# ethanshenley/Neural-Collaborative-Filtering-Demo

Measured on AMD Instinct MI355X. Metric: train samples/sec + infer pairs/sec, 1M×100K d=64 AdvancedNCF @1/2/4/8 GPU, higher is better.
Workload: dtype fp32; 1 GPU; C2 train step: 1M users x 100K items, D=64, H=4, MLP [256,128,64], T=32, dropout 0.2, Adam lr 1e-3 wd 1e-5 (dense-exact); global_batch=20480, groups_per_gpu=4096, samples_per_group=5, launch=host launches, parallelism=single-gpu

## Files before the change

neural-collaborative-filtering-demo_amd/csrc/dedup.hip:

```cpp
#include "segments.h"

using namespace ncf_seg;

namespace {

constexpr uint32_t ST_AGG = 1u << 30, ST_INCL = 2u << 30, ST_MASK = (1u << 30) - 1;
constexpr int kDirectTiles = 64;

__device__ __forceinline__ uint32_t ld_status(const uint32_t* p) {
  return __hip_atomic_load(p, __ATOMIC_RELAXED, __HIP_MEMORY_SCOPE_AGENT);
}
__device__ __forceinline__ void st_status(uint32_t* p, uint32_t v) {
  __hip_atomic_store(p, v, __ATOMIC_RELAXED, __HIP_MEMORY_SCOPE_AGENT);
}
__device__ __forceinline__ uint64_t ld_status64(const uint64_t* p) {
  return __hip_atomic_load(p, __ATOMIC_RELAXED, __HIP_MEMORY_SCOPE_AGENT);
}
__device__ __forceinline__ void st_status64(uint64_t* p, uint64_t v) {
  __hip_atomic_store(p, v, __ATOMIC_RELAXED, __HIP_MEMORY_SCOPE_AGENT);
}

__device__ __forceinline__ uint32_t clamp_key(int64_t id, int64_t rows) {
  return (id < 0 || id >= rows) ? 0u : (uint32_t)id;
}

__global__ __launch_bounds__(256) void k_keys_hist(
    const int64_t* __restrict__ ids0, int64_t rows0, const int64_t* __restrict__ ids1,
    int64_t rows1, int64_t n0, int64_t n1, int bits, int passes, uint32_t* __restrict__ k0,
    uint32_t* __restrict__ v0, uint32_t* __restrict__ k1, uint32_t* __restrict__ v1,
    uint32_t* __restrict__ ghist, uint32_t* __restrict__ num_unique, uint32_t* __restrict__ start0,
    uint32_t* __restrict__ start1, uint32_t* __restrict__ pstart0, uint32_t* __restrict__ pstart1,
    uint32_t* __restrict__ fpiece0, uint32_t* __restrict__ fpiece1) {
  __shared__ uint32_t h[MAXP][MAXR];
  const int kind = blockIdx.y;
  const int64_t n = kind ? n1 : n0;
  const int64_t rows = kind ? rows1 : rows0;
  const int64_t* ids = kind ? ids1 : ids0;
  uint32_t* k = kind ? k1 : k0;
  uint32_t* v = kind ? v1 : v0;
  const int R = 1 << bits;
  if (n == 0) {
    if (blockIdx.x == 0 && threadIdx.x == 0) {
      if (num_unique) num_unique[kind] = 0;
      (kind ? start1 : start0)[0] = 0;
      (kind ? pstart1 : pstart0)[0] = 0;
      (kind ? fpiece1 : fpiece0)[0] = 0;
    }
    return;
  }
  if ((int64_t)blockIdx.x * TILE >= n) return;
  for (int i = threadIdx.x; i < passes * MAXR; i += 256) (&h[0][0])[i] = 0;
  __syncthreads();
#pragma unroll
  for (int r = 0; r < 4; ++r) {
    const int64_t i = (int64_t)blockIdx.x * TILE + r * 256 + threadIdx.x;
    if (i < n) {
      const uint32_t key = clamp_key(ids[i], rows);
      k[i] = key;
      v[i] = (uint32_t)i;
      for (int p = 0; p < passes; ++p) atomicAdd(&h[p][(key >> (p * bits)) & (R - 1)], 1u);
    }
  }
  __syncthreads();
  for (int p = 0; p < passes; ++p)
    for (int d = threadIdx.x; d < R; d += 256)
      if (h[p][d]) atomicAdd(&ghist[((int64_t)p * 2 + kind) * MAXR + d], h[p][d]);
}

__global__ __launch_bounds__(256) void k_onesweep(
    const uint32_t* __restrict__ kin0, const uint32_t* __restrict__ vin0,
    const uint32_t* __restrict__ kin1, const uint32_t* __restrict__ vin1, int64_t n0, int64_t n1,
    int shift, int bits, const uint32_t* __restrict__ ghist, uint32_t* __restrict__ status,
    int nbmax, uint32_t* __restrict__ tickets, uint32_t* __restrict__ kout0,
    uint32_t* __restrict__ vout0, uint32_t* __restrict__ kout1, uint32_t* __restrict__ vout1) {
  __shared__ uint32_t wcnt[4][MAXR];
  __shared__ uint32_t tcnt[MAXR];
  __shared__ uint32_t base[MAXR];
  __shared__ uint32_t csum[256];
  __shared__ uint32_t s_tile;
  const int kind = blockIdx.y;
  const int64_t n = kind ? n1 : n0;
  if (n == 0) return;
  const int nb = (int)((n + TILE - 1) / TILE);
  const int R = 1 << bits;
  const int tid = threadIdx.x, lane = tid & 63, w = tid >> 6;
  if (tid == 0) s_tile = atomicAdd(&tickets[kind], 1u);
  for (int i = tid; i < 4 * R; i += 256) wcnt[i / R][i % R] = 0;
  __syncthreads();
  const int tile = (int)s_tile;
  if (tile >= nb) return;
  const uint32_t* kin = kind ? kin1 : kin0;
  const uint32_t* vin = kind ? vin1 : vin0;
  uint32_t* kout = kind ? kout1 : kout0;
  uint32_t* vout = kind ? vout1 : vout0;
  uint32_t* st = status + ((int64_t)kind * nbmax) * R;

  const int64_t kb = (int64_t)tile * TILE + w * 256;
  uint32_t key[4], val[4], dig[4], loc[4];
  bool ok[4];
  const uint64_t lt = (lane == 0) ? 0ull : ((~0ull) >> (64 - lane));
#pragma unroll
  for (int it = 0; it < 4; ++it) {
    const int64_t i = kb + it * 64 + lane;
    ok[it] = i < n;
    key[it] = ok[it] ? kin[i] : 0u;
    val[it] = ok[it] ? vin[i] : 0u;
    dig[it] = (key[it] >> shift) & (uint32_t)(R - 1);
    uint64_t peers = __ballot(ok[it]);
    for (int b = 0; b < bits; ++b) {
      const uint64_t bb = __ballot((dig[it] >> b) & 1u);
      peers &= ((dig[it] >> b) & 1u) ? bb : ~bb;
    }
    const uint32_t before = (uint32_t)__popcll(peers & lt);
    uint32_t c = 0;
    if (ok[it]) c = wcnt[w][dig[it]];
    __builtin_amdgcn_wave_barrier();
    loc[it] = c + before;
    if (ok[it] && before == 0) wcnt[w][dig[it]] = c + (uint32_t)__popcll(peers);
    __builtin_amdgcn_wave_barrier();
  }
  __syncthreads();
  for (int d = tid; d < R; d += 256) {
    uint32_t run = 0;
#pragma unroll
    for (int ww = 0; ww < 4; ++ww) {
      const uint32_t c = wcnt[ww][d];
      wcnt[ww][d] = run;
      run += c;
    }
    tcnt[d] = run;
    st_status(&st[(int64_t)tile * R + d], (tile == 0 ? ST_INCL : ST_AGG) | run);
  }
  const uint32_t* gh = ghist + (int64_t)kind * MAXR;
  const int per = (R + 255) / 256;
  uint32_t mine = 0;
  for (int j = 0; j < per; ++j) {
    const int d = tid * per + j;
    if (d < R) mine += gh[d];
  }
  csum[tid] = mine;
  __syncthreads();
  for (int off = 1; off < 256; off <<= 1) {
    const uint32_t x = tid >= off ? csum[tid - off] : 0u;
    __syncthreads();
    csum[tid] += x;
    __syncthreads();
  }
  {
    uint32_t run = csum[tid] - mine;
    for (int j = 0; j < per; ++j) {
      const int d = tid * per + j;
      if (d < R) {
        base[d] = run;
        run += gh[d];
      }
    }
  }
  __syncthreads();
  if (nb <= kDirectTiles) {
    const uint64_t* st64 = reinterpret_cast<const uint64_t*>(st);
    for (int d0 = 2 * tid; d0 < R; d0 += 512) {
      uint32_t e0 = 0, e1 = 0;
      for (int tb = 0; tb < tile; tb += 8) {
        uint64_t v[8];
#pragma unroll
        for (int j = 0; j < 8; ++j)
          v[j] = tb + j < tile ? ld_status64(&st64[((int64_t)(tb + j) * R + d0) / 2])
                               : ((uint64_t)ST_AGG << 32 | ST_AGG);
#pragma unroll
        for (int j = 0; j < 8; ++j) {
          while (((uint32_t)v[j] & ~ST_MASK) == 0 || ((uint32_t)(v[j] >> 32) & ~ST_MASK) == 0) {
            __builtin_amdgcn_s_sleep(1);
            v[j] = ld_status64(&st64[((int64_t)(tb + j) * R + d0) / 2]);
          }
          e0 += (uint32_t)v[j] & ST_MASK;
          e1 += (uint32_t)(v[j] >> 32) & ST_MASK;
        }
      }
      base[d0] += e0;
      base[d0 + 1] += e1;
    }
  } else {
    for (int d = tid; d < R; d += 256) {
      uint32_t excl = 0;
      if (tile > 0) {
        int t = tile - 1;
        while (true) {
          const uint32_t s = ld_status(&st[(int64_t)t * R + d]);
          if ((s & ~ST_MASK) == 0) {
            __builtin_amdgcn_s_sleep(1);
            continue;
          }
          excl += s & ST_MASK;
          if (s & ST_INCL) break;
          --t;
        }
        st_status(&st[(int64_t)tile * R + d], ST_INCL | (excl + tcnt[d]));
      }
      base[d] += excl;
    }
  }
  __syncthreads();
#pragma unroll
  for (int it = 0; it < 4; ++it) {
    if (!ok[it]) continue;
    const uint32_t pos = base[dig[it]] + wcnt[w][dig[it]] + loc[it];
    kout[pos] = key[it];
    vout[pos] = val[it];
  }
}

__global__ __launch_bounds__(256) void k_segments(
    const uint32_t* __restrict__ sk0, const uint32_t* __restrict__ sk1, int64_t n0, int64_t n1,
    int nbmax, uint64_t* __restrict__ sstatus, uint32_t* __restrict__ tickets,
    uint32_t* __restrict__ segoff, uint32_t* __restrict__ start0, uint32_t* __restrict__ start1,
    uint32_t* __restrict__ pstart0, uint32_t* __restrict__ pstart1, uint32_t* __restrict__ pseg0,
    uint32_t* __restrict__ pseg1, uint32_t* __restrict__ fpiece0, uint32_t* __restrict__ fpiece1,
    int64_t* __restrict__ uniq0, int64_t* __restrict__ uniq1, int32_t* __restrict__ slot0,
    int32_t* __restrict__ slot1, uint32_t* __restrict__ totals, uint32_t* __restrict__ num_unique) {
  constexpr uint64_t F_AGG = 1ull << 62, F_INCL = 2ull << 62, M31 = (1ull << 31) - 1;
  __shared__ uint32_t ws_s[16], ws_p[16];
  __shared__ uint32_t s_tile, s_es, s_ep;
  const int kind = blockIdx.y;
  const int64_t n = kind ? n1 : n0;
  if (n == 0) return;
  const int nb = (int)((n + TILE - 1) / TILE);
  const int tid = threadIdx.x, lane = tid & 63, w = tid >> 6;
  if (tid == 0) s_tile = atomicAdd(&tickets[kind], 1u);
  __syncthreads();
  const int tile = (int)s_tile;
  if (tile >= nb) return;
  const uint32_t* sk = kind ? sk1 : sk0;
  uint64_t* st = sstatus + (int64_t)kind * nbmax;
  const uint64_t le = (lane == 63) ? ~0ull : ((1ull << (lane + 1)) - 1);
  bool sh[4], ph[4];
  uint32_t sr[4], pr[4], key[4];
#pragma unroll
  for (int r = 0; r < 4; ++r) {
    const int64_t i = (int64_t)tile * TILE + r * 256 + tid;
    key[r] = i < n ? sk[i] : 0u;
    sh[r] = i < n && (i == 0 || key[r] != sk[i - 1]);
    ph[r] = i < n && (sh[r] || (i % PIECE) == 0);
    const uint64_t ms = __ballot(sh[r]), mp = __ballot(ph[r]);
    sr[r] = (uint32_t)__popcll(ms & le);
    pr[r] = (uint32_t)__popcll(mp & le);
    if (lane == 0) {
      ws_s[r * 4 + w] = (uint32_t)__popcll(ms);
      ws_p[r * 4 + w] = (uint32_t)__popcll(mp);
    }
  }
  __syncthreads();
  if (w == 0) {
    uint64_t S = 0, Pc = 0;
    for (int q = 0; q < 16; ++q) { S += ws_s[q]; Pc += ws_p[q]; }
    uint64_t es = 0, ep = 0;
    if (nb <= kDirectTiles) {
      if (lane == 0) st_status64(&st[tile], F_AGG | (S << 31) | Pc);
      uint64_t v = 0;
      if (lane < tile) {
        do {
          v = ld_status64(&st[lane]);
          if ((v >> 62) == 0) __builtin_amdgcn_s_sleep(1);
        } while ((v >> 62) == 0);
      }
      uint32_t a = (uint32_t)((v >> 31) & M31), b = (uint32_t)(v & M31);
#pragma unroll
      for (int o = 32; o > 0; o >>= 1) {
        a += __shfl_xor(a, o, 64);
        b += __shfl_xor(b, o, 64);
      }
      es = a;
      ep = b;
    } else if (lane == 0) {
      if (tile == 0) {
        st_status64(&st[0], F_INCL | (S << 31) | Pc);
      } else {
        st_status64(&st[tile], F_AGG | (S << 31) | Pc);
        int t = tile - 1;
        while (true) {
          const uint64_t s = ld_status64(&st[t]);
          if ((s >> 62) == 0) {
            __builtin_amdgcn_s_sleep(1);
            continue;
          }
          es += (s >> 31) & M31;
          ep += s & M31;
          if (s & F_INCL) break;
          --t;
        }
// ... 155 lines not shown
}

static int64_t g_small_max = kSmallMax;

__global__ __launch_bounds__(256) void k_seg_inverse(const uint32_t* __restrict__ sk0,
                                                     const uint32_t* __restrict__ sk1,
                                                     const uint32_t* __restrict__ sv0,
                                                     const uint32_t* __restrict__ sv1, int64_t n0,
                                                     int64_t n1, int nb,
                                                     const uint32_t* __restrict__ off,
                                                     int64_t* __restrict__ inv0,
                                                     int64_t* __restrict__ inv1) {
  __shared__ uint32_t wsum[16];
  const int kind = blockIdx.y;
  const int64_t n = kind ? n1 : n0;
  const uint32_t* sk = kind ? sk1 : sk0;
  const uint32_t* sv = kind ? sv1 : sv0;
  int64_t* inv = kind ? inv1 : inv0;
  const int lane = threadIdx.x & 63, w = threadIdx.x >> 6;
  bool head[4];
  uint32_t rank[4];
  const uint64_t le = (lane == 63) ? ~0ull : ((1ull << (lane + 1)) - 1);
  for (int r = 0; r < 4; ++r) {
    const int64_t i = (int64_t)blockIdx.x * TILE + r * 256 + threadIdx.x;
    head[r] = i < n && (i == 0 || sk[i] != sk[i - 1]);
    const uint64_t m = __ballot(head[r]);
    rank[r] = (uint32_t)__popcll(m & le);
    if (lane == 0) wsum[r * 4 + w] = (uint32_t)__popcll(m);
  }
  __syncthreads();
  const uint32_t base = off[(int64_t)kind * nb + blockIdx.x];
  for (int r = 0; r < 4; ++r) {
    const int64_t i = (int64_t)blockIdx.x * TILE + r * 256 + threadIdx.x;
    if (i >= n) continue;
    uint32_t pre = 0;
    for (int q = 0; q < r * 4 + w; ++q) pre += wsum[q];
    inv[sv[i]] = (int64_t)(base + pre + rank[r]) - 1;
  }
}

}

extern "C" int ncf_dedup_ids2(const int64_t* ids0, int64_t n0, int64_t rows0, const int64_t* ids1,
                              int64_t n1, int64_t rows1, int64_t dim, int64_t* uniq0,
                              int64_t* uniq1, int32_t* slot0, int32_t* slot1,
                              uint32_t* num_unique, void* workspace, int64_t workspace_bytes,
                              void* stream) {
  const int64_t n = n0 > n1 ? n0 : n1;
  NCF_CHECK_ARG(n0 >= 0 && n1 >= 0 && n < (1ll << 30), "ncf_dedup_ids: bad n");
  NCF_CHECK_ARG(rows0 >= 1 && rows1 >= 1 && rows0 <= (1ll << 32) && rows1 <= (1ll << 32),
                "ncf_dedup_ids: rows must be in [1, 2^32]");
  if (workspace_bytes < ws_bytes(n, dim)) {
    ncf_set_error("ncf_dedup_ids: workspace %lld < %lld bytes", (long long)workspace_bytes,
                  (long long)ws_bytes(n, dim));
    return NCF_ERR_WORKSPACE;
  }
  hipStream_t st = (hipStream_t)stream;
  WS w = carve(workspace, n, dim);
  const int passes = sort_passes(rows0, rows1), bits = digit_bits(rows0, rows1);
  if (n == 0) {
    if (num_unique) (void)hipMemsetAsync(num_unique, 0, 2 * sizeof(uint32_t), st);
    (void)hipMemsetAsync(w.totals, 0, 4 * sizeof(uint32_t), st);
    return NCF_OK;
  }
  if (n <= g_small_max) {
    uint32_t *k0, *v0, *k1, *v1;
    sorted_bufs(w, passes, &k0, &v0, &k1, &v1);
    hipLaunchKernelGGL(k_dedup_small, dim3(1, 2), dim3(1024), 0, st, ids0, rows0, ids1, rows1, n0,
                       n1, w.nb, k0, v0, k1, v1, w.segoff, w.start0, w.start1, w.pstart0,
                       w.pstart1, w.pseg0, w.pseg1, w.fpiece0, w.fpiece1, uniq0, uniq1, slot0,
                       slot1, w.totals, num_unique);
    NCF_CHECK_LAUNCH("ncf_dedup_ids(small)");
    return NCF_OK;
  }
  (void)hipMemsetAsync(workspace, 0, (size_t)w.zero_bytes(workspace, passes, bits), st);
  hipLaunchKernelGGL(k_keys_hist, dim3(w.nb, 2), dim3(256), 0, st, ids0, rows0, ids1, rows1, n0,
                     n1, bits, passes, w.ka0, w.va0, w.ka1, w.va1, w.ghist, num_unique, w.start0,
                     w.start1, w.pstart0, w.pstart1, w.fpiece0, w.fpiece1);
  NCF_CHECK_LAUNCH("ncf_dedup_ids(keys)");
  uint32_t *ki0 = w.ka0, *vi0 = w.va0, *ki1 = w.ka1, *vi1 = w.va1;
  uint32_t *ko0 = w.kb0, *vo0 = w.vb0, *ko1 = w.kb1, *vo1 = w.vb1;
  const int64_t R = 1ll << bits;
  for (int p = 0; p < passes; ++p) {
    hipLaunchKernelGGL(k_onesweep, dim3(w.nb, 2), dim3(256), 0, st, ki0, vi0, ki1, vi1, n0, n1,
                       p * bits, bits, w.ghist + (int64_t)p * 2 * MAXR,
                       w.status + (int64_t)p * 2 * w.nb * R, w.nb, w.tickets + 2 * p, ko0, vo0,
                       ko1, vo1);
    NCF_CHECK_LAUNCH("ncf_dedup_ids(sort)");
    uint32_t* t;
    t = ki0; ki0 = ko0; ko0 = t;
    t = vi0; vi0 = vo0; vo0 = t;
    t = ki1; ki1 = ko1; ko1 = t;
    t = vi1; vi1 = vo1; vo1 = t;
  }
  hipLaunchKernelGGL(k_segments, dim3(w.nb, 2), dim3(256), 0, st, ki0, ki1, n0, n1, w.nb,
                     w.sstatus, w.tickets + 2 * MAXP, w.segoff, w.start0, w.start1, w.pstart0,
                     w.pstart1, w.pseg0, w.pseg1, w.fpiece0, w.fpiece1, uniq0, uniq1,
                     slot0, slot1, w.totals, num_unique);
  NCF_CHECK_LAUNCH("ncf_dedup_ids(segments)");
  return NCF_OK;
}

extern "C" int ncf_dedup_ids(const int64_t* user_ids, const int64_t* item_ids, int64_t n,
                             int64_t dim, int64_t num_users, int64_t num_items,
                             int64_t* uniq_users, int64_t* uniq_items, int32_t* slot_users,
                             int32_t* slot_items, uint32_t* num_unique, void* workspace,
                             int64_t workspace_bytes, void* stream) {
  return ncf_dedup_ids2(user_ids, n, num_users, item_ids, n, num_items, dim, uniq_users,
                        uniq_items, slot_users, slot_items, num_unique, workspace,
                        workspace_bytes, stream);
}

extern "C" int64_t ncf_embedding_bwd_workspace(int64_t n, int64_t dim) { return ws_bytes(n, dim); }

extern "C" int64_t ncf_dedup_set_small_max(int64_t n) {
  const int64_t prev = g_small_max;
  if (n >= 0) g_small_max = n < kSmallMax ? n : kSmallMax;
  return prev;
}

extern "C" int ncf_dedup_inverse(int64_t n0, int64_t n1, int64_t rows0, int64_t rows1, int64_t dim,
                                 int64_t* inv0, int64_t* inv1, void* workspace,
                                 int64_t workspace_bytes, void* stream) {
  const int64_t n = n0 > n1 ? n0 : n1;
  if (workspace_bytes < ws_bytes(n, dim)) {
    ncf_set_error("ncf_dedup_inverse: workspace too small");
    return NCF_ERR_WORKSPACE;
  }
  if (n == 0) return NCF_OK;
  WS w = carve(workspace, n, dim);
  uint32_t *k0, *v0, *k1, *v1;
  sorted_bufs(w, sort_passes(rows0, rows1), &k0, &v0, &k1, &v1);
  hipLaunchKernelGGL(k_seg_inverse, dim3(w.nb, 2), dim3(256), 0, (hipStream_t)stream, k0, k1, v0,
                     v1, n0, n1, w.nb, w.segoff, inv0, inv1);
  NCF_CHECK_LAUNCH("ncf_dedup_inverse");
  return NCF_OK;
}
```

neural-collaborative-filtering-demo_amd/csrc/mlp_tower_dev.h:

```cpp
#pragma once
#include "ncf_common.h"

namespace ncf_mlp {
namespace {

#ifndef NCF_BWD_RING
#define NCF_BWD_RING 4
#endif
#ifndef NCF_MLP_RT
#define NCF_MLP_RT 5
#endif
constexpr int kRT = NCF_MLP_RT;
constexpr int kRows = 16 * kRT;
constexpr int kThreads = 512;
constexpr int kWaves = kThreads / 64;
constexpr int kPQ = 260;
constexpr int kPP = 132;
constexpr int N0 = 256, N1 = 128, N2 = 64;
constexpr int kPSize = kRows * kPP > kWaves * 3 * N0 ? kRows * kPP : kWaves * 3 * N0;
template <int K0>
struct Lay {
  static constexpr int kHmfW = 0, kHmfB = K0, kHmlW = K0 + 4, kHmlB = kHmlW + N2, kHfW = kHmlB + 4,
                       kHfB = kHfW + 4, kHloss = kHfB + 4;
  static constexpr int kHeadW = kHloss + 4;
// ... 881 lines not shown
  const uint64_t cs = clock ? clock->seed : 0ull;
  using T = Lay<K0>;
  constexpr int WM = MM == 3 ? 0 : MM;
  float* pp = part + (int64_t)blockIdx.x * T::kPartW;
  NCF_STAMP(1, 0);
  if (fused_head) {
    head_bwd<K0>(Q, P, row0, rows, h, a.l[2], p, a.seed[2] + cs, inv_n, pp + 3 * (N0 + N1 + N2));
  } else {
    for (int e = threadIdx.x; e < kRows * (N2 / 4); e += kThreads) {
      const int r = e / (N2 / 4), c = (e % (N2 / 4)) * 4;
      lds4_st(Q + r * kPQ + c,
              r < rows ? ld4(g_last + (row0 + r) * N2 + c) : make_float4(0.f, 0.f, 0.f, 0.f));
    }
    __syncthreads();
  }
  NCF_STAMP(1, 1);
  ln_bwd<N2, kPQ>(Q, P, row0, rows, a.l[2], p, a.seed[2] + cs, pp);
  NCF_STAMP(1, 2);
  float* R1 = nullptr;
  if (fused_wgrad) {
    stage_act<N1, kPP>(P, a.l[1], row0, rows, p, a.seed[1] + cs, R1);
    __syncthreads();
    NCF_STAMP(1, 3);
    wgrad_layer<N2, N1, kPQ, kPP, WM>(Q, P, pp + T::kW2);
    __syncthreads();
    NCF_STAMP(1, 4);
  }
  lin_bwd<N2, N1, kPQ, kPP, MM>(Q, P, a.l[2].w, a.l[2].ldw);
  __syncthreads();
  NCF_STAMP(1, 5);
  ln_bwd<N1, kPP>(P, Q, row0, rows, a.l[1], p, a.seed[1] + cs, pp + 3 * N2, R1);
  NCF_STAMP(1, 6);
  if (fused_wgrad) {
    stage_act<N0, kPQ>(Q, a.l[0], row0, rows, p, a.seed[0] + cs);
    __syncthreads();
    NCF_STAMP(1, 7);
    wgrad_layer<N1, N0, kPP, kPQ, WM>(P, Q, pp + T::kW1);
    __syncthreads();
    NCF_STAMP(1, 8);
  }
  lin_bwd<N1, N0, kPP, kPQ, MM>(P, Q, a.l[1].w, a.l[1].ldw);
  __syncthreads();
  NCF_STAMP(1, 9);
  ln_bwd<N0, kPQ>(Q, P, row0, rows, a.l[0], p, a.seed[0] + cs, pp + 3 * (N2 + N1));
  NCF_STAMP(1, 10);
  if (fused_wgrad) {
    stage_rows<K0, kPP>(P, xin, row0, rows);
    __syncthreads();
    NCF_STAMP(1, 11);
    wgrad_layer<N0, K0, kPQ, kPP, WM>(Q, P, pp + T::kW0);
    __syncthreads();
    NCF_STAMP(1, 12);
  }
  lin_bwd<N0, K0, kPQ, kPP, MM>(Q, P, a.l[0].w, a.l[0].ldw);
  __syncthreads();
  NCF_STAMP(1, 13);
  if (dx) {
    for (int e = threadIdx.x; e < rows * (K0 / 4); e += kThreads) {
      const int r = e / (K0 / 4), c = (e % (K0 / 4)) * 4;
      st4(dx + (row0 + r) * K0 + c, lds4(P + r * kPP + c));
    }
  }
#ifdef NCF_MLP_STAMPS
  __syncthreads();
#endif
  NCF_STAMP(1, 14);
}

template <int K0, int MM = 0>
__global__ __launch_bounds__(kThreads) void k_mlp_bwd(const float* __restrict__ g_last, int64_t n,
                                                      TowerArgs a, float p,
                                                      const ncf_step_clock* clock,
                                                      float* __restrict__ dx,
                                                      float* __restrict__ part, ncf_head_args h,
                                                      int fused_head, float inv_n,
                                                      const float* __restrict__ xin, int fused_wgrad) {
  extern __shared__ float lds[];
  mlp_bwd_body<K0, MM>(lds, g_last, n, a, p, clock, dx, part, h, fused_head, inv_n, xin,
                       fused_wgrad);
}

constexpr size_t kLds = sizeof(float) * (kRows * kPQ + kPSize);
constexpr size_t kLdsFwd = sizeof(float) * 16 * kFwdRT * (kPQ + kPP);
static_assert(kWaves * 3 * N0 <= kPSize, "ln_bwd scratch must fit in buffer P");
static_assert(kWaves * Lay<128>::kHeadW <= kPSize, "head scratch must fit in buffer P");
static_assert(kWaves * 3 * N1 <= kRows * kPQ, "ln_bwd scratch of layer 1 must fit in buffer Q");
static_assert(128 <= kPP - 4, "a 128-wide input fits buffer P");

bool tower_ok(int64_t dim, int64_t n_layers, const int64_t* hidden) {
  return (dim == 64 || dim == 128) && n_layers == 3 && hidden && hidden[0] == N0 &&
         hidden[1] == N1 && hidden[2] == N2;
}

int make_args(const ncf_mlp_layer* layers, uint64_t seed, int64_t dim, TowerArgs& a) {
  for (int l = 0; l < 3; ++l) {
    a.l[l] = layers[l];
    if (!a.l[l].w || !a.l[l].b || !a.l[l].gamma || !a.l[l].beta || a.l[l].ldw < (l ? 0 : dim) ||
        (a.l[l].ldw & 3)) {
      ncf_set_error("ncf_mlp: layer %d needs w/b/gamma/beta and a float4-aligned ldw", l);
      return NCF_ERR_ARG;
    }
    a.seed[l] = (seed + 0x9E37ull * (uint64_t)(l + 1)) & 0x7FFFFFFFFFFFFFFFull;
  }
  return NCF_OK;
}

template <int K0>
int defer_tower(const TowerArgs& a, const ncf_head_args* head, const ncf_head_args& h,
                       float inv_n, bool fw, int nb, float* workspace, ncf_reduce_list* lst) {
  using T = Lay<K0>;
  constexpr int PW = T::kPartW;
  int rc = NCF_OK;
  const int widths[3] = {N0, N1, N2};
  const int64_t offs[3] = {3 * (N2 + N1), 3 * N2, 0};
  for (int l = 0; l < 3 && !rc; ++l) {
    const int W = widths[l];
    const float* pp = workspace + offs[l];
    const ncf_mlp_layer& L = a.l[l];
    const ptrdiff_t s1 = L.dgamma - L.dbias, s2 = L.dbeta - L.dgamma;
    if (s1 == s2 && s1 >= W) {
      rc = ncf_defer(lst, pp, nb, PW, 3 * W, L.dbias, 0, W, s1);
    } else {
      rc = ncf_defer(lst, pp, nb, PW, W, L.dbias, 0, W, W);
      if (!rc) rc = ncf_defer(lst, pp + W, nb, PW, W, L.dgamma, 0, W, W);
      if (!rc) rc = ncf_defer(lst, pp + 2 * W, nb, PW, W, L.dbeta, 0, W, W);
    }
  }
  if (!rc && fw) {
    rc = ncf_defer(lst, workspace + T::kW0, nb, PW, N0 * K0, a.l[0].dw, 0, K0, a.l[0].ldw);
    if (!rc) rc = ncf_defer(lst, workspace + T::kW1, nb, PW, N1 * N0, a.l[1].dw, 0, N0, a.l[1].ldw);
    if (!rc) rc = ncf_defer(lst, workspace + T::kW2, nb, PW, N2 * N1, a.l[2].dw, 0, N1, a.l[2].ldw);
  }
  if (!rc && head) {
    const float* hp = workspace + 3 * (N0 + N1 + N2);
    float* base = h.grad_mf_out_w;
    const bool flat = h.grad_mf_out_b == base + T::kHmfB && h.grad_mlp_out_w == base + T::kHmlW &&
                      h.grad_mlp_out_b == base + T::kHmlB && h.grad_final_w == base + T::kHfW &&
                      h.grad_final_b == base + T::kHfB;
    if (flat) {
      rc = ncf_defer(lst, hp, nb, PW, T::kHfB + 1, base, 0, T::kHfB + 1, T::kHfB + 1);
    } else {
      rc = ncf_defer(lst, hp + T::kHmfW, nb, PW, K0, h.grad_mf_out_w, 0, K0, K0);
      if (!rc) rc = ncf_defer(lst, hp + T::kHmfB, nb, PW, 1, h.grad_mf_out_b, 0, 1, 1);
      if (!rc) rc = ncf_defer(lst, hp + T::kHmlW, nb, PW, N2, h.grad_mlp_out_w, 0, N2, N2);
      if (!rc) rc = ncf_defer(lst, hp + T::kHmlB, nb, PW, 1, h.grad_mlp_out_b, 0, 1, 1);
      if (!rc) rc = ncf_defer(lst, hp + T::kHfW, nb, PW, 2, h.grad_final_w, 0, 2, 2);
      if (!rc) rc = ncf_defer(lst, hp + T::kHfB, nb, PW, 1, h.grad_final_b, 0, 1, 1);
    }
    if (!rc && h.loss) rc = ncf_defer(lst, hp + T::kHloss, nb, PW, 1, h.loss, 0, 1, 1, inv_n);
  }
  return rc;
}

}
}
```

neural-collaborative-filtering-demo_amd/csrc/ncf_common.h:

```cpp
#pragma once
#include <hip/hip_runtime.h>
#include <stdint.h>
#include <string.h>
#include <stdio.h>
#include <stdlib.h>

#include "ncf_hip.h"

#define NCF_WAVE 64

void ncf_set_error(const char* fmt, ...);


#define NCF_CHECK_ARG(cond, ...)                 \
  do {                                           \
    if (!(cond)) {                               \
      ncf_set_error(__VA_ARGS__);                \
      return NCF_ERR_ARG;                        \
    }                                            \
  } while (0)

static inline bool ncf_debug_sync() {
  static int on = -1;
  if (on < 0) {
    const char* e = getenv("NCF_DEBUG_SYNC");
    on = (e && e[0] == '1') ? 1 : 0;
  }
  return on != 0;
}

#define NCF_CHECK_LAUNCH(name)                                                   \
  do {                                                                           \
    hipError_t e_ = hipGetLastError();                                           \
    if (e_ == hipSuccess && ncf_debug_sync()) {                                  \
      e_ = hipDeviceSynchronize();                                               \
      if (e_ != hipSuccess) {                                                    \
        fprintf(stderr, "NCF_DEBUG_SYNC: %s: %s\n", name, hipGetErrorString(e_)); \
        fflush(stderr);                                                          \
      }                                                                          \
    }                                                                            \
    if (e_ != hipSuccess) {                                                      \
      ncf_set_error("%s: launch failed: %s", name, hipGetErrorString(e_));       \
      return NCF_ERR_LAUNCH;                                                     \
    }                                                                            \
  } while (0)

static inline int ncf_cdiv(int64_t a, int64_t b) { return (int)((a + b - 1) / b); }

template <int L>
__device__ __forceinline__ float group_sum(float v) {
#pragma unroll
  for (int o = L / 2; o > 0; o >>= 1) v += __shfl_xor(v, o, 64);
  return v;
}

__device__ __forceinline__ float wave_sum(float v) { return group_sum<64>(v); }

__device__ __forceinline__ float4 ld4(const float* p) { return *reinterpret_cast<const float4*>(p); }
__device__ __forceinline__ void st4(float* p, float4 v) { *reinterpret_cast<float4*>(p) = v; }

__device__ __forceinline__ float ncf_bf2f(uint32_t h) { return __uint_as_float(h << 16); }
__device__ __forceinline__ uint32_t ncf_f2bf(float f) {
  return __builtin_bit_cast(uint16_t, (__bf16)f);
}
__device__ __forceinline__ float ncf_round_bf16(float f) { return (float)(__bf16)f; }
template <bool BF>
__device__ __forceinline__ float ldp(const float* p, int64_t i) {
  if constexpr (BF) return ncf_bf2f(reinterpret_cast<const uint16_t*>(p)[i]);
  else return p[i];
}
template <bool BF>
__device__ __forceinline__ void stp(float* p, int64_t i, float v) {
  if constexpr (BF) reinterpret_cast<uint16_t*>(p)[i] = (uint16_t)ncf_f2bf(v);
  else p[i] = v;
}
template <bool BF>
__device__ __forceinline__ float4 ldp4(const float* p, int64_t i) {
  if constexpr (BF) {
    const uint2 r = *reinterpret_cast<const uint2*>(reinterpret_cast<const uint16_t*>(p) + i);
    return make_float4(__uint_as_float(r.x << 16), __uint_as_float(r.x & 0xffff0000u),
                       __uint_as_float(r.y << 16), __uint_as_float(r.y & 0xffff0000u));
  } else {
    return ld4(p + i);
  }
}
template <bool BF>
__device__ __forceinline__ void stp4(float* p, int64_t i, float4 v) {
  if constexpr (BF) {
    uint2 r;
    r.x = ncf_f2bf(v.x) | (ncf_f2bf(v.y) << 16);
    r.y = ncf_f2bf(v.z) | (ncf_f2bf(v.w) << 16);
    *reinterpret_cast<uint2*>(reinterpret_cast<uint16_t*>(p) + i) = r;
// ... 138 lines not shown
```

neural-collaborative-filtering-demo_amd/csrc/reduce.hip:

```cpp
#include "ncf_common.h"

namespace {

constexpr int kPB = 64;
constexpr int kMaxPerLaunch = 24;
int VEC_LANES = 1;

struct BatchArgs {
  ncf_reduce_desc d[kMaxPerLaunch];
  int64_t scr[kMaxPerLaunch];
  uint32_t first[kMaxPerLaunch + 1];
  int32_t chunks[kMaxPerLaunch];
  int32_t vec[kMaxPerLaunch];
  int32_t count;
};

__device__ __forceinline__ int find_desc(const BatchArgs& a, uint32_t b) {
  int i = 0;
  while (i + 1 < a.count && a.first[i + 1] <= b) ++i;
  return i;
}

__device__ __forceinline__ void store_out(const ncf_reduce_desc& d, int64_t i, float t) {
  float* o = d.out + (i / d.cols) * d.ldo + (i % d.cols);
  const float v = d.scale * t;
  *o = d.accumulate ? *o + v : v;
}

template <typename T> __device__ __forceinline__ T zero();
template <> __device__ __forceinline__ float zero<float>() { return 0.0f; }
template <> __device__ __forceinline__ float4 zero<float4>() { return make_float4(0.f, 0.f, 0.f, 0.f); }

template <typename T>
__device__ __forceinline__ T stage1_sum(const float* __restrict__ part, int64_t stride, int64_t i,
                                        int pb, int pe, int w) {
  T a0 = zero<T>(), a1 = zero<T>(), a2 = zero<T>(), a3 = zero<T>();
  int p = pb + w;
  for (; p + 60 < pe; p += 64) {
    T v[16];
#pragma unroll
    for (int j = 0; j < 16; ++j) v[j] = *(const T*)(part + (int64_t)(p + 4 * j) * stride + i);
#pragma unroll
    for (int j = 0; j < 16; j += 4) {
      a0 += v[j];
      a1 += v[j + 1];
      a2 += v[j + 2];
      a3 += v[j + 3];
    }
  }
  for (; p + 12 < pe; p += 16) {
    a0 += *(const T*)(part + (int64_t)p * stride + i);
    a1 += *(const T*)(part + (int64_t)(p + 4) * stride + i);
    a2 += *(const T*)(part + (int64_t)(p + 8) * stride + i);
    a3 += *(const T*)(part + (int64_t)(p + 12) * stride + i);
  }
  for (; p < pe; p += 4) a0 += *(const T*)(part + (int64_t)p * stride + i);
  return (a0 + a1) + (a2 + a3);
}

__global__ __launch_bounds__(256) void k_reduce_batch1(const BatchArgs a, float* __restrict__ scratch) {
  __shared__ float4 red[4][64];
  const int di = find_desc(a, blockIdx.x);
  const ncf_reduce_desc& d = a.d[di];
  const int ch = a.chunks[di];
  const bool vec = a.vec[di] != 0;
  const int vw = vec ? 4 : 1;
  const uint32_t local = blockIdx.x - a.first[di];
  const uint32_t gx = (uint32_t)((d.L + 64 * vw - 1) / (64 * vw));
  const int64_t i = ((int64_t)(local % gx) * 64 + (threadIdx.x & 63)) * vw;
  const int y = (int)(local / gx);
  const int w = threadIdx.x >> 6;
  const int l = threadIdx.x & 63;
  const int pb = ch > 1 ? y * kPB : 0;
  const int pe = ch > 1 ? min(d.P, pb + kPB) : d.P;
  if (vec) {
    float4 s = zero<float4>();
    if (i < d.L) s = stage1_sum<float4>(d.part, d.stride, i, pb, pe, w);
    red[w][l] = s;
    __syncthreads();
    if (w == 0 && i < d.L) {
      const float4 t = (red[0][l] + red[1][l]) + (red[2][l] + red[3][l]);
      if (ch > 1) {
        *(float4*)(scratch + a.scr[di] + (int64_t)y * d.L + i) = t;
      } else {
        store_out(d, i, t.x);
        store_out(d, i + 1, t.y);
        store_out(d, i + 2, t.z);
        store_out(d, i + 3, t.w);
      }
    }
    return;
  }
  float s = 0.0f;
  if (i < d.L) s = stage1_sum<float>(d.part, d.stride, i, pb, pe, w);
  red[w][l].x = s;
  __syncthreads();
  if (w == 0 && i < d.L) {
    const float t = (red[0][l].x + red[1][l].x) + (red[2][l].x + red[3][l].x);
    if (ch > 1) scratch[a.scr[di] + (int64_t)y * d.L + i] = t;
    else store_out(d, i, t);
  }
}

template <typename T>
__device__ __forceinline__ T stage2_sum(const float* __restrict__ s, int64_t L, int pe) {
  T ws[4];
#pragma unroll
  for (int w = 0; w < 4; ++w) {
    T a0 = zero<T>(), a1 = zero<T>(), a2 = zero<T>(), a3 = zero<T>();
    int p = w;
    for (; p + 12 < pe; p += 16) {
      a0 += *(const T*)(s + (int64_t)p * L);
      a1 += *(const T*)(s + (int64_t)(p + 4) * L);
      a2 += *(const T*)(s + (int64_t)(p + 8) * L);
      a3 += *(const T*)(s + (int64_t)(p + 12) * L);
    }
    for (; p < pe; p += 4) a0 += *(const T*)(s + (int64_t)p * L);
    ws[w] = (a0 + a1) + (a2 + a3);
  }
  return (ws[0] + ws[1]) + (ws[2] + ws[3]);
}

__global__ __launch_bounds__(256) void k_reduce_batch2(const BatchArgs a,
                                                       const float* __restrict__ scratch) {
  const int di = find_desc(a, blockIdx.x);
  const ncf_reduce_desc& d = a.d[di];
  const bool vec = a.vec[di] != 0;
  const int64_t i = ((int64_t)(blockIdx.x - a.first[di]) * 256 + threadIdx.x) * (vec ? 4 : 1);
  if (i >= d.L) return;
  const float* s = scratch + a.scr[di] + i;
  const int pe = a.chunks[di];
  if (vec) {
    const float4 t = stage2_sum<float4>(s, d.L, pe);
    store_out(d, i, t.x);
    store_out(d, i + 1, t.y);
    store_out(d, i + 2, t.z);
    store_out(d, i + 3, t.w);
    return;
  }
  store_out(d, i, stage2_sum<float>(s, d.L, pe));
}

int chunks_of(int P) { return P > NCF_REDUCE_ONE_STAGE ? (P + kPB - 1) / kPB : 1; }

}

extern "C" int64_t ncf_reduce_set_vec(int64_t on) {
  const int was = VEC_LANES;
  if (on >= 0) VEC_LANES = on > 0 ? 1 : 0;
  return was;
}

extern "C" int64_t ncf_reduce_batch_scratch(const ncf_reduce_list* list) {
  if (!list) return 0;
  int64_t f = 0;
  for (int i = 0; i < list->count && i < NCF_REDUCE_LIST_MAX; ++i) {
    const int c = chunks_of(list->d[i].P);
    if (c > 1) f += (int64_t)c * list->d[i].L;
  }
  return f;
}

extern "C" int ncf_reduce_batch(const ncf_reduce_list* list, float* scratch,
                                int64_t scratch_floats, void* stream) {
  NCF_CHECK_ARG(list && list->count >= 0 && list->count <= NCF_REDUCE_LIST_MAX,
                "ncf_reduce_batch: bad list");
  if (scratch_floats < ncf_reduce_batch_scratch(list)) {
    ncf_set_error("ncf_reduce_batch: scratch %lld < %lld floats", (long long)scratch_floats,
                  (long long)ncf_reduce_batch_scratch(list));
    return NCF_ERR_WORKSPACE;
  }
  hipStream_t st = (hipStream_t)stream;
  int64_t scr_off = 0;
  for (int base = 0; base < list->count; base += kMaxPerLaunch) {
    BatchArgs a1, a2;
    memset(&a1, 0, sizeof(a1));
    memset(&a2, 0, sizeof(a2));
    uint32_t b1 = 0, b2 = 0;
    for (int j = 0; j < kMaxPerLaunch && base + j < list->count; ++j) {
      const ncf_reduce_desc& d = list->d[base + j];
      NCF_CHECK_ARG(d.part && d.out && d.L >= 0 && d.P >= 1 && d.cols >= 1 && d.stride >= d.L,
                    "ncf_reduce_batch: bad descriptor %d", base + j);
      const int c = chunks_of(d.P);
      const bool vec = VEC_LANES > 0 && d.L % 4 == 0 && d.stride % 4 == 0 &&
                       ((uintptr_t)d.part & 15) == 0 &&
                       (c == 1 || (scr_off % 4 == 0 && ((uintptr_t)scratch & 15) == 0));
      const int vw = vec ? 4 : 1;
      const uint32_t gx = (uint32_t)((d.L + 64 * vw - 1) / (64 * vw));
      a1.d[a1.count] = d;
      a1.vec[a1.count] = vec;
      a1.chunks[a1.count] = c;
      a1.first[a1.count] = b1;
      a1.scr[a1.count] = c > 1 ? scr_off : 0;
      b1 += gx * (uint32_t)c;
      if (c > 1) {
        a2.d[a2.count] = d;
        a2.chunks[a2.count] = c;
        a2.vec[a2.count] = vec;
        a2.first[a2.count] = b2;
        a2.scr[a2.count] = scr_off;
        b2 += (uint32_t)((d.L + 256 * vw - 1) / (256 * vw));
        ++a2.count;
// ... 18 lines not shown
```

neural-collaborative-filtering-demo_amd/csrc/tower_fused.hip:

```cpp
#include "attn_block_dev.h"
#include "mlp_tower_dev.h"

#ifndef NCF_TF
#define NCF_TF(name) name
#endif

namespace {

namespace A = ncf_attn;
namespace T = ncf_mlp;

constexpr int kD = 64, kM = 5;
constexpr int kGW = A::AG<kD>::kGroups;
constexpr int kVR = kGW * kM;
constexpr int kRp = 16 * ((kGW * kM + 15) / 16);
static_assert(kVR <= T::kRows && kRp == T::kRows, "the attention groups fill the tower tile");
static_assert(A::kThreads == T::kThreads, "one workgroup shape");
constexpr size_t kAttnFwdFloats = 3 * kRp * A::AG<kD>::kPitch + kGW * 8 * A::kMaxM +
                                  16 * A::AG<kD>::kPitch;
constexpr bool kAttnInQ = kAttnFwdFloats <= (size_t)T::kRows * T::kPQ;
constexpr size_t kAttnFwdOff = kAttnInQ ? 0 : T::kLdsFwd / sizeof(float);

template <int HD, int MM>
__global__ __launch_bounds__(T::kThreads) void k_attn_mlp_fwd(
    const float* __restrict__ xu, const float* __restrict__ xi, int64_t B,
    const float* __restrict__ wq, const float* __restrict__ bq, const float* __restrict__ wk,
    const float* __restrict__ bk, const float* __restrict__ wv, const float* __restrict__ bv,
    const float* __restrict__ wo, const float* __restrict__ bo, float scale, float p_drop,
    uint64_t seed, const ncf_step_clock* clock, float* __restrict__ Q, float* __restrict__ K,
    float* __restrict__ V, float* __restrict__ P, float* __restrict__ Y,
    const int64_t* __restrict__ uids, T::TowerArgs a, float eps,
    const float* __restrict__ w_out, const float* __restrict__ b_out,
    const float* __restrict__ mf_pred, const float* __restrict__ w_fin,
    const float* __restrict__ b_fin, float* __restrict__ mlp_pred, float* __restrict__ prob) {
  extern __shared__ float lds[];
  float* x_tile = lds + T::kRows * T::kPQ;
  A::attn_block_fwd_body<kD, HD>(lds + kAttnFwdOff, xu, xi, B, kM, wq, bq, wk, bk, wv, bv, wo, bo,
                                 scale, p_drop, seed, clock, Q, K, V, P, nullptr, Y, 1, uids,
                                 A::kShareQ, x_tile, T::kPP);
  __syncthreads();
  T::mlp_fwd_body<kD, T::kRT, kVR, MM>(lds, Y, B * kM, a, eps, p_drop, clock, w_out, b_out,
                                       mf_pred, w_fin, b_fin, mlp_pred, prob, true);
}

template <int HD, int MM>
__global__ __launch_bounds__(T::kThreads) void k_attn_mlp_bwd(
    int64_t B, T::TowerArgs a, float p_drop, const ncf_step_clock* clock,
    float* __restrict__ part_tower, ncf_head_args h, float inv_n, const float* __restrict__ Y,
    const float* __restrict__ Qg, const float* __restrict__ Kg, const float* __restrict__ Vg,
    const float* __restrict__ Pg, const float* __restrict__ wq, const float* __restrict__ wk,
    const float* __restrict__ wv, const float* __restrict__ wo, float scale, uint64_t seed,
    const float* __restrict__ xu, const float* __restrict__ xi, float* __restrict__ part_attn,
    float* __restrict__ dxu, float* __restrict__ dxi, const int64_t* __restrict__ uids) {
  extern __shared__ float lds[];
  T::mlp_bwd_body<kD, MM, kVR>(lds, nullptr, B * kM, a, p_drop, clock, nullptr, part_tower, h, 1,
                               inv_n, Y, 1);
  __syncthreads();
  A::attn_block_bwd_body<kD, HD, false, false>(lds, nullptr, Qg, Kg, Vg, Pg, B, kM, wq, wk, wv, wo, scale,
                                        p_drop, seed, clock, nullptr, xu, xi, part_attn, nullptr,
                                        nullptr, nullptr, dxu, dxi, nullptr, nullptr, nullptr, uids,
                                        A::kShareQ, lds + T::kRows * T::kPQ, T::kPP);
}

constexpr size_t kLdsFused = T::kLdsFwd + (kAttnInQ ? 0 : sizeof(float) * kAttnFwdFloats);
constexpr size_t kLdsFusedBwd = T::kLds;
static_assert(sizeof(float) * (5 * kRp * A::AG<kD>::kPitch + kGW * 8 * kM * kM) <= kLdsFusedBwd,
              "the attention backward (8 heads at most) fits the tower backward's LDS");
static_assert(kRp * A::AG<kD>::kPitch <= T::kRows * T::kPQ,
              "the attention backward's dY copy (S0) lies below the tower's dX tile");

int64_t tf_workspace(int64_t groups, int which) {
  const int64_t nb = groups <= 0 ? 1 : ncf_cdiv(groups, kGW);
  if (which == 0) {
    constexpr int W = T::Lay<128>::kPartW;
    return nb * W + 2 * ncf_reduce_scratch((int)nb, W);
  }
  constexpr int64_t PA = A::AG<kD>::kPartAttn;
  return nb * PA + ncf_reduce_scratch((int)nb, (int)PA) * 4;
}

}

extern "C" int64_t NCF_TF(ncf_attn_mlp_bwd_workspace)(int64_t groups, int32_t which) {
  return tf_workspace(groups, which);
}

extern "C" int NCF_TF(ncf_attn_mlp_fused_supported)(int64_t dim, int64_t heads, int64_t group_len,
                                                    int64_t n_layers, const int64_t* hidden) {
  return dim == kD && group_len == kM && heads >= 1 && dim % heads == 0 && dim / heads <= 16 &&
                 A::hd_ok(dim, dim / heads) && T::tower_ok(dim, n_layers, hidden)
             ? 1
             : 0;
}

extern "C" int NCF_TF(ncf_attn_mlp_fwd)(const float* xu, const float* xi, int64_t groups, int64_t heads,
                                const float* wq, const float* bq, const float* wk, const float* bk,
                                const float* wv, const float* bv, const float* wo, const float* bo,
                                float dropout_p, uint64_t seed, const ncf_step_clock* clock,
                                float* q, float* k, float* v, float* probs, float* y,
                                const int64_t* user_ids, const ncf_mlp_layer* layers,
                                int64_t n_layers, const int64_t* hidden, float eps,
                                const float* mlp_out_w, const float* mlp_out_b,
                                const float* mf_pred, const float* final_w, const float* final_b,
                                float* mlp_pred, float* prob, int32_t tower_mode, void* stream) {
  NCF_CHECK_ARG(groups >= 0 && NCF_TF(ncf_attn_mlp_fused_supported)(kD, heads, kM, n_layers, hidden),
                "ncf_attn_mlp_fwd: unsupported shape (need D = 64, M = 5, hidden [256,128,64])");
  NCF_CHECK_ARG(dropout_p >= 0.0f && dropout_p < 1.0f, "ncf_attn_mlp_fwd: dropout_p out of [0,1)");
  NCF_CHECK_ARG(q && k && v && probs && y, "ncf_attn_mlp_fwd: the training stash (q, k, v, probs) "
                "and y are required");
  NCF_CHECK_ARG(tower_mode == 0 || tower_mode == 1 || tower_mode == 3,
                "ncf_attn_mlp_fwd: tower_mode 0, 1 or 3");
  if (groups == 0) return NCF_OK;
  T::TowerArgs a;
  const int rc = T::make_args(layers, seed, kD, a);
  if (rc) return rc;
  hipStream_t st = (hipStream_t)stream;
  const float scale = sqrtf((float)(kD / heads));
  const dim3 grid((unsigned)ncf_cdiv(groups, kGW));
#define NCF_FUSED_FWD(HD_, MM_)                                                                   \
  if (kD / heads == HD_ && tower_mode == MM_) {                                                   \
    static bool attr = false;                                                                     \
    if (!attr) {                                                                                  \
      (void)hipFuncSetAttribute((const void*)k_attn_mlp_fwd<HD_, MM_>,                            \
                                hipFuncAttributeMaxDynamicSharedMemorySize, (int)kLdsFused);      \
      attr = true;                                                                                \
    }                                                                                             \
    hipLaunchKernelGGL((k_attn_mlp_fwd<HD_, MM_>), grid, dim3(T::kThreads), kLdsFused, st, xu, xi,  \
                       groups, wq, bq, wk, bk, wv, bv, wo, bo, scale, dropout_p, seed, clock, q, k, \
                       v, probs, y, user_ids, a, eps, mlp_out_w, mlp_out_b, mf_pred, final_w,     \
                       final_b, mlp_pred, prob);                                                  \
  }
  NCF_FUSED_FWD(8, 0) NCF_FUSED_FWD(16, 0)
  NCF_FUSED_FWD(8, 1) NCF_FUSED_FWD(16, 1)
  NCF_FUSED_FWD(8, 3) NCF_FUSED_FWD(16, 3)
#undef NCF_FUSED_FWD
  NCF_CHECK_LAUNCH("ncf_attn_mlp_fwd");
  return NCF_OK;
}

extern "C" int NCF_TF(ncf_attn_mlp_bwd)(int64_t groups, int64_t heads, const float* y,
                                const ncf_mlp_layer* layers, int64_t n_layers,
                                const int64_t* hidden, float dropout_p, uint64_t seed,
                                const ncf_step_clock* clock, const ncf_head_args* head,
                                float* tower_workspace, int64_t tower_workspace_floats,
                                const float* q, const float* k, const float* v, const float* probs,
                                const float* wq, const float* wk, const float* wv, const float* wo,
                                const float* xu, const float* xi, float* const* attn_grad_params,
                                float* attn_workspace, int64_t attn_workspace_floats,
// ... 64 lines not shown
```

Before: 77.13 million samples/s.

## Shrink onesweep LDS with 16-bit counts and batch stage-2 reduce loads

The radix onesweep kernel moves from static to dynamic shared memory sized by the digit width, and stores per-wave and per-tile digit counts as 16-bit values. This lets a sort tile fit on a CU next to a tower workgroup, so the sort can co-reside with the tower kernels and can run at more workgroups per CU. Static asserts tie the tower LDS budgets to a shared constant. Separately, the stage-2 reduction now issues batches of up to 64 independent loads before accumulating, to raise memory-level parallelism, at the cost of more registers and a changed summation order.

```diff
diff --git a/neural-collaborative-filtering-demo_amd/csrc/dedup.hip b/neural-collaborative-filtering-demo_amd/csrc/dedup.hip
--- a/neural-collaborative-filtering-demo_amd/csrc/dedup.hip
+++ b/neural-collaborative-filtering-demo_amd/csrc/dedup.hip
@@ -67,25 +67,36 @@
       if (h[p][d]) atomicAdd(&ghist[((int64_t)p * 2 + kind) * MAXR + d], h[p][d]);
 }
 
+constexpr size_t onesweep_lds(int bits) {
+  return ((size_t)4 + 4 * 2 + 2) * ((size_t)1 << bits) + 4 * 256 + 4;
+}
+static_assert(TILE <= 65535, "k_onesweep keeps its in-tile digit counts in 16 bits");
+static_assert(onesweep_lds(MAX_BITS) <= 36864,
+              "k_onesweep at the widest digit must fit the LDS a tower workgroup leaves free");
+static_assert(NCF_TOWER_LDS + onesweep_lds(MAX_BITS) <= NCF_CU_LDS,
+              "a sort tile must fit on a CU beside a tower workgroup");
+
 __global__ __launch_bounds__(256) void k_onesweep(
     const uint32_t* __restrict__ kin0, const uint32_t* __restrict__ vin0,
     const uint32_t* __restrict__ kin1, const uint32_t* __restrict__ vin1, int64_t n0, int64_t n1,
     int shift, int bits, const uint32_t* __restrict__ ghist, uint32_t* __restrict__ status,
     int nbmax, uint32_t* __restrict__ tickets, uint32_t* __restrict__ kout0,
     uint32_t* __restrict__ vout0, uint32_t* __restrict__ kout1, uint32_t* __restrict__ vout1) {
-  __shared__ uint32_t wcnt[4][MAXR];
-  __shared__ uint32_t tcnt[MAXR];
-  __shared__ uint32_t base[MAXR];
-  __shared__ uint32_t csum[256];
-  __shared__ uint32_t s_tile;
+  extern __shared__ uint32_t sweep_lds[];
+  const int R = 1 << bits;
+  uint32_t* const base = sweep_lds;
+  uint32_t* const csum = base + R;
+  uint32_t& s_tile = csum[256];
+  uint16_t* const wcnt0 = reinterpret_cast<uint16_t*>(csum + 257);
+  uint16_t* const tcnt = wcnt0 + 4 * R;
   const int kind = blockIdx.y;
   const int64_t n = kind ? n1 : n0;
   if (n == 0) return;
   const int nb = (int)((n + TILE - 1) / TILE);
-  const int R = 1 << bits;
   const int tid = threadIdx.x, lane = tid & 63, w = tid >> 6;
+  uint16_t* const wc = wcnt0 + w * R;
   if (tid == 0) s_tile = atomicAdd(&tickets[kind], 1u);
-  for (int i = tid; i < 4 * R; i += 256) wcnt[i / R][i % R] = 0;
+  for (int i = tid; i < 2 * R; i += 256) reinterpret_cast<uint32_t*>(wcnt0)[i] = 0;
   __syncthreads();
   const int tile = (int)s_tile;
   if (tile >= nb) return;
@@ -113,10 +124,10 @@
     }
     const uint32_t before = (uint32_t)__popcll(peers & lt);
     uint32_t c = 0;
-    if (ok[it]) c = wcnt[w][dig[it]];
+    if (ok[it]) c = wc[dig[it]];
     __builtin_amdgcn_wave_barrier();
     loc[it] = c + before;
-    if (ok[it] && before == 0) wcnt[w][dig[it]] = c + (uint32_t)__popcll(peers);
+    if (ok[it] && before == 0) wc[dig[it]] = (uint16_t)(c + (uint32_t)__popcll(peers));
     __builtin_amdgcn_wave_barrier();
   }
   __syncthreads();
@@ -124,11 +135,11 @@
     uint32_t run = 0;
 #pragma unroll
     for (int ww = 0; ww < 4; ++ww) {
-      const uint32_t c = wcnt[ww][d];
-      wcnt[ww][d] = run;
+      const uint32_t c = wcnt0[ww * R + d];
+      wcnt0[ww * R + d] = (uint16_t)run;
       run += c;
     }
-    tcnt[d] = run;
+    tcnt[d] = (uint16_t)run;
     st_status(&st[(int64_t)tile * R + d], (tile == 0 ? ST_INCL : ST_AGG) | run);
   }
   const uint32_t* gh = ghist + (int64_t)kind * MAXR;
@@ -204,7 +215,7 @@
 #pragma unroll
   for (int it = 0; it < 4; ++it) {
     if (!ok[it]) continue;
-    const uint32_t pos = base[dig[it]] + wcnt[w][dig[it]] + loc[it];
+    const uint32_t pos = base[dig[it]] + wc[dig[it]] + loc[it];
     kout[pos] = key[it];
     vout[pos] = val[it];
   }
@@ -526,7 +537,8 @@
   uint32_t *ko0 = w.kb0, *vo0 = w.vb0, *ko1 = w.kb1, *vo1 = w.vb1;
   const int64_t R = 1ll << bits;
   for (int p = 0; p < passes; ++p) {
-    hipLaunchKernelGGL(k_onesweep, dim3(w.nb, 2), dim3(256), 0, st, ki0, vi0, ki1, vi1, n0, n1,
+    hipLaunchKernelGGL(k_onesweep, dim3(w.nb, 2), dim3(256), onesweep_lds(bits), st, ki0, vi0, ki1,
+                       vi1, n0, n1,
                        p * bits, bits, w.ghist + (int64_t)p * 2 * MAXR,
                        w.status + (int64_t)p * 2 * w.nb * R, w.nb, w.tickets + 2 * p, ko0, vo0,
                        ko1, vo1);
diff --git a/neural-collaborative-filtering-demo_amd/csrc/mlp_tower_dev.h b/neural-collaborative-filtering-demo_amd/csrc/mlp_tower_dev.h
--- a/neural-collaborative-filtering-demo_amd/csrc/mlp_tower_dev.h
+++ b/neural-collaborative-filtering-demo_amd/csrc/mlp_tower_dev.h
@@ -987,6 +987,8 @@
 
 constexpr size_t kLds = sizeof(float) * (kRows * kPQ + kPSize);
 constexpr size_t kLdsFwd = sizeof(float) * 16 * kFwdRT * (kPQ + kPP);
+static_assert(kLds <= NCF_TOWER_LDS && kLdsFwd <= NCF_TOWER_LDS,
+              "the id sort is sized to the LDS a tower workgroup leaves free (ncf_common.h)");
 static_assert(kWaves * 3 * N0 <= kPSize, "ln_bwd scratch must fit in buffer P");
 static_assert(kWaves * Lay<128>::kHeadW <= kPSize, "head scratch must fit in buffer P");
 static_assert(kWaves * 3 * N1 <= kRows * kPQ, "ln_bwd scratch of layer 1 must fit in buffer Q");
diff --git a/neural-collaborative-filtering-demo_amd/csrc/ncf_common.h b/neural-collaborative-filtering-demo_amd/csrc/ncf_common.h
--- a/neural-collaborative-filtering-demo_amd/csrc/ncf_common.h
+++ b/neural-collaborative-filtering-demo_amd/csrc/ncf_common.h
@@ -8,6 +8,9 @@
 #include "ncf_hip.h"
 
 #define NCF_WAVE 64
+
+constexpr size_t NCF_CU_LDS = 160 * 1024;
+constexpr size_t NCF_TOWER_LDS = 125440;
 
 void ncf_set_error(const char* fmt, ...);
 
diff --git a/neural-collaborative-filtering-demo_amd/csrc/reduce.hip b/neural-collaborative-filtering-demo_amd/csrc/reduce.hip
--- a/neural-collaborative-filtering-demo_amd/csrc/reduce.hip
+++ b/neural-collaborative-filtering-demo_amd/csrc/reduce.hip
@@ -104,20 +104,38 @@
 
 template <typename T>
 __device__ __forceinline__ T stage2_sum(const float* __restrict__ s, int64_t L, int pe) {
+  constexpr int kBatch = sizeof(T) == sizeof(float) ? 64 : 32;
+  T a[4][4];
+#pragma unroll
+  for (int w = 0; w < 4; ++w)
+#pragma unroll
+    for (int k = 0; k < 4; ++k) a[w][k] = zero<T>();
+  for (int b = 0; b < pe; b += kBatch) {
+    T v[kBatch];
+#pragma unroll
+    for (int g = 0; g < kBatch; g += 16) {
+      if (b + g < pe) {
+#pragma unroll
+        for (int j = 0; j < 16; ++j)
+          v[g + j] = *(const T*)(s + (int64_t)min(b + g + j, pe - 1) * L);
+      }
+    }
+#pragma unroll
+    for (int g = 0; g < kBatch; g += 16) {
+      if (b + g < pe) {
+#pragma unroll
+        for (int j = 0; j < 16; ++j) {
+          const int w = j & 3, k = j >> 2;
+          const bool full = b + g + w + 12 < pe;
+          if (full) a[w][k] += v[g + j];
+          else if (b + g + j < pe) a[w][0] += v[g + j];
+        }
+      }
+    }
+  }
   T ws[4];
 #pragma unroll
-  for (int w = 0; w < 4; ++w) {
-    T a0 = zero<T>(), a1 = zero<T>(), a2 = zero<T>(), a3 = zero<T>();
-    int p = w;
-    for (; p + 12 < pe; p += 16) {
-      a0 += *(const T*)(s + (int64_t)p * L);
-      a1 += *(const T*)(s + (int64_t)(p + 4) * L);
-      a2 += *(const T*)(s + (int64_t)(p + 8) * L);
-      a3 += *(const T*)(s + (int64_t)(p + 12) * L);
-    }
-    for (; p < pe; p += 4) a0 += *(const T*)(s + (int64_t)p * L);
-    ws[w] = (a0 + a1) + (a2 + a3);
-  }
+  for (int w = 0; w < 4; ++w) ws[w] = (a[w][0] + a[w][1]) + (a[w][2] + a[w][3]);
   return (ws[0] + ws[1]) + (ws[2] + ws[3]);
 }
 
diff --git a/neural-collaborative-filtering-demo_amd/csrc/tower_fused.hip b/neural-collaborative-filtering-demo_amd/csrc/tower_fused.hip
--- a/neural-collaborative-filtering-demo_amd/csrc/tower_fused.hip
+++ b/neural-collaborative-filtering-demo_amd/csrc/tower_fused.hip
@@ -64,6 +64,8 @@
 
 constexpr size_t kLdsFused = T::kLdsFwd + (kAttnInQ ? 0 : sizeof(float) * kAttnFwdFloats);
 constexpr size_t kLdsFusedBwd = T::kLds;
+static_assert(kLdsFused <= NCF_TOWER_LDS && kLdsFusedBwd <= NCF_TOWER_LDS,
+              "the id sort is sized to the LDS a fused tower workgroup leaves free (ncf_common.h)");
 static_assert(sizeof(float) * (5 * kRp * A::AG<kD>::kPitch + kGW * 8 * kM * kM) <= kLdsFusedBwd,
               "the attention backward (8 heads at most) fits the tower backward's LDS");
 static_assert(kRp * A::AG<kD>::kPitch <= T::kRows * T::kPQ,
```

After: 78.33 million samples/s, median of 6. 1.6% higher.
